# CVMI-Lab/HybridNeuralRendering

Hardware: AMD Instinct MI355X
Metric: rays/sec (fwd render) scene0241_01 at 1/2/4/8 GPU; PSNR delta vs ref (higher is better)
Workload: dtype f32

## Files before the change

hybridneuralrendering_amd/csrc/mlp.hip:

```cpp
#include <stdlib.h>

#include "hnr_h2.h"
#include "hnr_launch.h"

namespace hnr {

constexpr int ML_PAD = 32;
constexpr int ML_SLOT = 8192 + ML_PAD;
constexpr int ML_WSTEP = 8192;
constexpr int ML_META_FLOATS = 4 * 128 + 4 + 4;
constexpr int ML_DESC = 4 * 128, ML_WMAX = 4 * 128 + 4;

struct MlpArgs {
    const float *A; int lda;
    const float *R; const int32_t *ridx; int ldr;
    const char *wimg;
    int wbase[4];
    int K0, N[4], act[4];
    float *C2; int ldc2;
    const float *loc_w; const int32_t *vs_item;
    const float *w2c, *Kmat, *campos, *campos_n;
    const float *fm; int H, W;
    const float *frame_w;
    const float *w_last, *b_last;
// ... 712 lines not shown
    for (int i = tid; i < MX_WBYTES / 16; i += 64 * MX_WAVES) {
        const int s = i >> 8, cp = (i >> 6) & 3, ln = i & 63;
        *reinterpret_cast<u32x4 *>(lds + i * 16) = *reinterpret_cast<const u32x4 *>(a.wimg + (size_t)s * ML_WSTEP + cp * 1024 + ln * 16);
    }
    for (int i = tid; i < 3 * 64; i += 64 * MX_WAVES) s_bias[i] = meta[(i >> 6) * 128 + (i & 63)];
    for (int i = tid; i < 3 * 128; i += 64 * MX_WAVES) s_fin[i] = a.w_fin[i];
    __syncthreads();
    const float dw0 = meta[ML_DESC + 0], dw1 = meta[ML_DESC + 1], dw2 = meta[ML_DESC + 2];
    const float bfin[3] = {a.b_fin[0], a.b_fin[1], a.b_fin[2]};
    const f32x2 slope2 = {a.slope, a.slope};
    for (int tile = blockIdx.x * MX_WAVES + wave; tile < n_tiles; tile += gridDim.x * MX_WAVES) {
        int lane = tid & 63;
        asm volatile("" : "+v"(lane));
        const int h = lane >> 5, j = lane & 31;
        const long long sbase = (long long)tile * 32;
        if (h == 0) s_max[j] = 0u;
        MW_WAVE_FENCE();
        float inv;
        float4 f4[12];
#pragma unroll
        for (int it = 0; it < 12; ++it) {
            const int idx = lane + 64 * it, row = idx / 24, q = idx - row * 24;
            long long sidx = sbase + row;
            if (sidx >= n_samp) sidx = n_samp - 1;
            if (q < 23) {
                f4[it] = *reinterpret_cast<const float4 *>(a.X7 + (size_t)sidx * a.ld7 + 4 * q);
            } else f4[it] = make_float4(0.f, 0.f, 0.f, 0.f);
        }
#pragma unroll
        for (int it = 0; it < 12; ++it) {
            const int idx = lane + 64 * it, row = idx / 24, q = idx - row * 24;
            if (q == 22) { f4[it].z = 0.f; f4[it].w = 0.f; }
            const float m = fmaxf(fmaxf(fabsf(f4[it].x), fabsf(f4[it].y)), fmaxf(fabsf(f4[it].z), fabsf(f4[it].w)));
            atomicMax(s_max + row, __float_as_uint(m));
        }
        MW_WAVE_FENCE();
        auto planes_half = [&](int half) {
#pragma unroll
            for (int it = 0; it < 12; ++it) {
                const int idx = lane + 64 * it, row = idx / 24, q = idx - row * 24, c = 4 * q - 48 * half;
                if (c >= 0 && c < 48) {
                    const float sc = pow2f(row_scale_exp(__uint_as_float(s_max[row])));
                    unsigned ph0, pm0, ph1, pm1;
                    split2h(__fmul_rn(f4[it].x, sc), __fmul_rn(f4[it].y, sc), ph0, pm0);
                    split2h(__fmul_rn(f4[it].z, sc), __fmul_rn(f4[it].w, sc), ph1, pm1);
                    char *dst = wl + (c >> 4) * MW_SLOT + ((((c >> 3) & 1) * 32 + row) * 16) + (c & 7) * 2;
                    *reinterpret_cast<uint2 *>(dst) = make_uint2(ph0, ph1);
                    *reinterpret_cast<uint2 *>(dst + 1024) = make_uint2(pm0, pm1);
                }
            }
        };
        planes_half(0);
        inv = __fmul_rn(pow2f(-row_scale_exp(__uint_as_float(s_max[j]))), dw0);
        MW_WAVE_FENCE();
        f32x16 acc[2];
        auto zero_acc = [&]() {
#pragma unroll
            for (int c = 0; c < 2; ++c)
#pragma unroll
                for (int r = 0; r < 16; ++r) acc[c][r] = 0.f;
        };
        auto activate = [&](int layer, bool act) -> float {
            float m = 0.f;
            const f32x2 inv2 = {inv, inv};
#pragma unroll
            for (int c = 0; c < 2; ++c) {
#pragma unroll
                for (int q4 = 0; q4 < 4; ++q4) {
                    const float4 b = *reinterpret_cast<const float4 *>(s_bias + layer * 64 + 32 * c + 16 * h + 4 * q4);
#pragma unroll
                    for (int e = 0; e < 2; ++e) {
                        const int q = 2 * q4 + e;
                        const f32x2 add = e ? f32x2{b.z, b.w} : f32x2{b.x, b.y};
                        f32x2 v = f32x2_fma(f32x2{acc[c][2 * q], acc[c][2 * q + 1]}, inv2, add);
                        if (act) { const f32x2 sv = v * slope2; v.x = fmaxf(v.x, sv.x); v.y = fmaxf(v.y, sv.y); }
                        acc[c][2 * q] = v.x; acc[c][2 * q + 1] = v.y;
                        m = fmaxf(fmaxf(m, fabsf(v.x)), fabsf(v.y));
                    }
                }
            }
            return m;
        };
        auto publish = [&](float dw, float m) {
            m = fmaxf(m, __shfl_xor(m, 32));
            const int k = row_scale_exp(m);
            const float sc = pow2f(k);
            const f32x2 sc2 = {sc, sc};
            inv = __fmul_rn(pow2f(-k), dw);
            MW_WAVE_FENCE();
#pragma unroll
            for (int c = 0; c < 2; ++c) {
                unsigned ph[8], pm[8];
#pragma unroll
                for (int q = 0; q < 8; ++q) {
                    const f32x2 vs = f32x2{acc[c][2 * q], acc[c][2 * q + 1]} * sc2;
                    split2h(vs.x, vs.y, ph[q], pm[q]);
                }
                if (2 * c + h < 3) {
                    char *dst = wl + (2 * c + h) * MW_SLOT + j * 16;
                    *reinterpret_cast<u32x4 *>(dst) = u32x4{ph[0], ph[1], ph[2], ph[3]};
                    *reinterpret_cast<u32x4 *>(dst + 512) = u32x4{ph[4], ph[5], ph[6], ph[7]};
                    *reinterpret_cast<u32x4 *>(dst + 1024) = u32x4{pm[0], pm[1], pm[2], pm[3]};
                    *reinterpret_cast<u32x4 *>(dst + 1024 + 512) = u32x4{pm[4], pm[5], pm[6], pm[7]};
                }
            }
            MW_WAVE_FENCE();
        };
        const char *wp = lds + lane * 16, *bp = wl + lane * 16;
        long long srow = sbase + j;
        const bool ok = srow < n_samp;
        if (!ok) srow = n_samp - 1;
        zero_acc();
        mw_layer<3>(wp, bp, acc);
        MW_WAVE_FENCE();
        planes_half(1);
        MW_WAVE_FENCE();
        mw_layer<3>(wp + 3 * 4096, bp, acc);
        publish(dw1, activate(0, true));
        zero_acc();
        mw_layer<3>(wp + 6 * 4096, bp, acc);
        publish(dw2, activate(1, true));
        const float *cfrow = a.CF + (size_t)srow * a.ldcf;
        float4 cfa[2][4], cfb[8];
#pragma unroll
        for (int c = 0; c < 2; ++c)
#pragma unroll
            for (int q4 = 0; q4 < 4; ++q4) cfa[c][q4] = *reinterpret_cast<const float4 *>(cfrow + 32 * c + 16 * h + 4 * q4);
#pragma unroll
        for (int q4 = 0; q4 < 8; ++q4) cfb[q4] = *reinterpret_cast<const float4 *>(cfrow + 64 + 32 * h + 4 * q4);
        zero_acc();
        mw_layer<3>(wp + 9 * 4096, bp, acc);
        (void)activate(2, false);
        if (a.Y && ok) {
            float *o = a.Y + (size_t)srow * a.ldy;
#pragma unroll
            for (int c = 0; c < 2; ++c)
#pragma unroll
                for (int q4 = 0; q4 < 4; ++q4) {
                    const int col = 32 * c + 16 * h + 4 * q4;
                    if (col + 4 <= 48) *reinterpret_cast<float4 *>(o + col) = make_float4(acc[c][4 * q4], acc[c][4 * q4 + 1], acc[c][4 * q4 + 2], acc[c][4 * q4 + 3]);
                }
        }
        float x[2][16];
#pragma unroll
        for (int c = 0; c < 2; ++c)
#pragma unroll
            for (int r = 0; r < 16; ++r) {
                const float cfv = reinterpret_cast<const float *>(&cfa[c][0])[r];
                x[c][r] = (32 * c + 16 * h + r < 45) ? acc[c][r] + cfv : cfv;
            }
        float rj[3];
#pragma unroll
        for (int o = 0; o < 3; ++o) {
            const float *wf = s_fin + o * 128;
            float pa[2][2];
#pragma unroll
            for (int c = 0; c < 2; ++c)
#pragma unroll
                for (int hf = 0; hf < 2; ++hf) {
                    float r = 0.f;
#pragma unroll
                    for (int e = 0; e < 8; ++e) r += x[c][8 * hf + e] * wf[32 * c + 16 * h + 8 * hf + e];
                    pa[c][hf] = r;
                }
            float pb[4];
#pragma unroll
            for (int i = 0; i < 4; ++i) {
                float r = 0.f;
#pragma unroll
                for (int e = 0; e < 8; ++e) r += reinterpret_cast<const float *>(&cfb[0])[8 * i + e] * wf[64 + 32 * h + 8 * i + e];
                pb[i] = r;
            }
            const float u0 = pa[0][0] + pa[0][1];
            const float u1 = pa[1][0] + pa[1][1];
            const float uh = (pb[0] + pb[1]) + (pb[2] + pb[3]);
            const float v0 = __shfl_xor(u0, 32), v1 = __shfl_xor(u1, 32), vh = __shfl_xor(uh, 32);
            const float lo = (u0 + v0) + (v1 + u1);
            const float hi = vh + uh;
            rj[o] = lo + hi;
        }
        if (ok && h == 0) {
            float4 out;
            out.x = a.sigma[srow];
#pragma unroll
            for (int o = 0; o < 3; ++o) {
                const float sg = hnr_div(1.f, 1.f + expf(-(rj[o] + bfin[o])));
                const float cch = sg * (1.f + 2.f * 0.001f) - 0.001f;
                if (o == 0) out.y = cch; else if (o == 1) out.z = cch; else out.w = cch;
            }
            reinterpret_cast<float4 *>(a.decoded)[a.vs_item[srow]] = out;
        }
        MW_WAVE_FENCE();
    }
}

struct MlpPackArgs {
    const float *W[4]; int ldw[4], N[4], K[4], S[4], base[4];
    const float *b[4];
    char *out; int total_steps;
};

__global__ void mlp_wmax_kernel(MlpPackArgs a)
{
    const int l = blockIdx.y;
    unsigned *wmax = reinterpret_cast<unsigned *>(a.out + (size_t)a.total_steps * ML_WSTEP) + ML_WMAX;
    float m = 0.f;
    for (int i = blockIdx.x * blockDim.x + threadIdx.x; i < a.N[l] * a.K[l]; i += gridDim.x * blockDim.x) {
        const int n = i / a.K[l], k = i - n * a.K[l];
        m = fmaxf(m, fabsf(a.W[l][(size_t)n * a.ldw[l] + k]));
    }
    for (int o = 32; o > 0; o >>= 1) m = fmaxf(m, __shfl_xor(m, o));
    if ((threadIdx.x & 63) == 0) atomicMax(wmax + l, __float_as_uint(m));
}

__global__ void mlp_pack_kernel(MlpPackArgs a)
{
    const int l = blockIdx.y;
    float *meta = reinterpret_cast<float *>(a.out + (size_t)a.total_steps * ML_WSTEP);
    const unsigned maxbits = reinterpret_cast<const unsigned *>(meta)[ML_WMAX + l];
    int ex = (int)((maxbits >> 23) & 0xffu);
    ex = ex < 110 ? 110 : (ex > 160 ? 160 : ex);
    const int sw = CH_W_EXP + 126 - ex;
    const float scale = pow2f(sw);
    const int total = a.S[l] * 4 * 64 * 8;
    for (int i = blockIdx.x * blockDim.x + threadIdx.x; i < total; i += gridDim.x * blockDim.x) {
        const int e = i & 7, ln = (i >> 3) & 63, ct = (i >> 9) & 3, s = i >> 11;
        const int ii = ln & 31, hh = ln >> 5;
        const int n = 32 * ct + 16 * ((ii >> 2) & 1) + (ii & 3) + 4 * (ii >> 3), k = 16 * s + 8 * hh + e;
        const float x = (n < a.N[l] && k < a.K[l]) ? __fmul_rn(a.W[l][(size_t)n * a.ldw[l] + k], scale) : 0.f;
        const _Float16 hv = (_Float16)x;
        const _Float16 mv = (_Float16)__fsub_rn(x, (float)hv);
        _Float16 *dst = reinterpret_cast<_Float16 *>(a.out + a.base[l] + (size_t)s * ML_WSTEP + (ct * 2) * 1024 + ln * 16) + e;
        dst[0] = hv;
        dst[512] = mv;
    }
    if (blockIdx.x == 0) {
        for (int i = threadIdx.x; i < 128; i += blockDim.x) meta[l * 128 + i] = (a.b[l] && i < a.N[l]) ? a.b[l][i] : 0.f;
        if (threadIdx.x == 0) meta[ML_DESC + l] = pow2f(-sw);
    }
}

}

using namespace hnr;

static int mlp_steps(int K) { return (K + 15) / 16; }

extern "C" int64_t hnr_mlp3_packed_bytes(int n_layers, const int *K)
{
    if (!K || (n_layers != 3 && n_layers != 4)) return -1;
    int64_t steps = 0;
    for (int l = 0; l < n_layers; ++l) { if (K[l] <= 0 || K[l] > 288) return -1; steps += mlp_steps(K[l]); }
    return steps * ML_WSTEP + ML_META_FLOATS * 4;
}

extern "C" int hnr_mlp3_pack(int n_layers, const float *const *d_W, const int *ldw, const int *N, const int *K, const float *const *d_bias, void *d_packed,
                             void *stream)
{
    if ((n_layers != 3 && n_layers != 4) || !d_W || !ldw || !N || !K || !d_bias || !d_packed || ((uintptr_t)d_packed & 15)) { set_error("hnr_mlp3_pack: NULL / unaligned pointer or n_layers not 3 / 4"); return HNR_ERR_BADARG; }
    MlpPackArgs a;
    int steps = 0;
    for (int l = 0; l < n_layers; ++l) {
        if (!d_W[l] || N[l] <= 0 || N[l] > 128 || K[l] <= 0 || K[l] > 288 || ldw[l] < K[l] || (l > 0 && K[l] != N[l == 3 ? 2 : l - 1])) {
            set_error("hnr_mlp3_pack: layer %d: N=%d (1..128) K=%d (1..288, = N of the layer it reads) ldw=%d", l, N[l], K[l], ldw[l]);
            return HNR_ERR_BADARG;
        }
        a.W[l] = d_W[l]; a.ldw[l] = ldw[l]; a.N[l] = N[l]; a.K[l] = K[l]; a.S[l] = mlp_steps(K[l]); a.b[l] = d_bias[l];
        a.base[l] = steps * ML_WSTEP;
        steps += a.S[l];
    }
    a.out = (char *)d_packed; a.total_steps = steps;
    hipStream_t st = (hipStream_t)stream;
    HNR_HIP_CHECK(hipMemsetAsync(a.out + (size_t)steps * ML_WSTEP, 0, ML_META_FLOATS * 4, st));
    mlp_wmax_kernel<<<dim3(16, n_layers), 256, 0, st>>>(a);
    HNR_LAUNCH_CHECK();
    mlp_pack_kernel<<<dim3(32, n_layers), 256, 0, st>>>(a);
    HNR_LAUNCH_CHECK();
    return HNR_OK;
}

static void mlp3_probe_print(hipStream_t st, int n_layers, int K0)
{
#ifdef HNR_MLP_PROBE
    if (knob_now("HNR_MLP_PROBE_PRINT", 0)) {
        (void)hipStreamSynchronize(st);
        long long h[24];
        if (hipMemcpyFromSymbol(h, HIP_SYMBOL(g_mlp_probe), sizeof(h)) == hipSuccess && h[20] > 0) {
            const char *nm[13] = {"wait/prev", "A load + split", "barrier", "L0 mfma", "L0 act", "L0 publish", "L1 mfma+act", "L1 publish", "L2 mfma", "L2 act", "store", "tail", "end barrier"};
            fprintf(stderr, "[mlp3 probe] n_layers %d K0 %d tiles %lld:", n_layers, K0, h[20]);
            for (int i = 0; i < 13; ++i) fprintf(stderr, " %s %lld", nm[i], h[i] / h[20]);
            fprintf(stderr, " [merge (a) %lld | tail: dot %lld, sigmoid %lld, loads %lld, merge+stores %lld]", h[13] / h[20], h[14] / h[20], h[15] / h[20], h[16] / h[20], h[17] / h[20]);
            fprintf(stderr, "\n");
        }
    }
#else
    (void)st; (void)n_layers; (void)K0;
#endif
}

static int mlp3_forward_impl(const float *d_A, int lda, int64_t M_cap, const int64_t *d_counts, int count_index, int count_mult, int seg_stride,
                             const void *d_packed, int n_layers, const int *N, const int *K, const int *act, float slope, const float *d_R,
                             const int32_t *d_ridx, int ldr, float *d_C, int ldc, float *d_C2, int ldc2, float *d_T0, int ldt0, float *d_T1, int ldt1,
                             uint32_t *d_tmax, void *stream);

extern "C" int hnr_mlp3_forward(const float *d_A, int lda, int64_t M_cap, const int64_t *d_counts, int count_index, int count_mult, int seg_stride,
                                const void *d_packed, int n_layers, const int *N, const int *K, const int *act, float slope, const float *d_R,
                                const int32_t *d_ridx, int ldr, float *d_C, int ldc, float *d_C2, int ldc2, void *stream)
{
    return mlp3_forward_impl(d_A, lda, M_cap, d_counts, count_index, count_mult, seg_stride, d_packed, n_layers, N, K, act, slope, d_R, d_ridx, ldr, d_C, ldc,
                             d_C2, ldc2, nullptr, 0, nullptr, 0, nullptr, stream);
}

namespace hnr {
int mlp3_forward_train(const float *d_A, int lda, int64_t M_cap, const int64_t *d_counts, int count_index, int count_mult, int seg_stride,
                       const void *d_packed, int n_layers, const int *N, const int *K, const int *act, float slope, const float *d_R,
                       const int32_t *d_ridx, int ldr, float *d_C, int ldc, float *d_C2, int ldc2, float *d_T0, int ldt0, float *d_T1, int ldt1,
                       uint32_t *d_tmax, void *stream)
{
    if (!d_T0 || !d_T1 || ldt0 < N[0] || ldt1 < N[1] || (ldt0 & 3) || (ldt1 & 3) || ((uintptr_t)d_T0 & 15) || ((uintptr_t)d_T1 & 15)) { set_error("mlp3_forward_train: bad activation buffers"); return HNR_ERR_BADARG; }
    return mlp3_forward_impl(d_A, lda, M_cap, d_counts, count_index, count_mult, seg_stride, d_packed, n_layers, N, K, act, slope, d_R, d_ridx, ldr, d_C, ldc,
                             d_C2, ldc2, d_T0, ldt0, d_T1, ldt1, d_tmax, stream);
}
}

static int mlp3_forward_impl(const float *d_A, int lda, int64_t M_cap, const int64_t *d_counts, int count_index, int count_mult, int seg_stride,
                             const void *d_packed, int n_layers, const int *N, const int *K, const int *act, float slope, const float *d_R,
                             const int32_t *d_ridx, int ldr, float *d_C, int ldc, float *d_C2, int ldc2, float *d_T0, int ldt0, float *d_T1, int ldt1,
                             uint32_t *d_tmax, void *stream)
{
    if ((n_layers != 3 && n_layers != 4) || !N || !K || !act || M_cap < 0 || seg_stride < 0 || (seg_stride > 0 && (count_mult < 1 || count_mult > 8)) || lda < K[0] || (lda & 3) || ldc < N[2] || (ldc & 3) ||
        !(slope > 0.f && slope < 1.f) || (d_R && (!d_ridx || ldr < N[0] || (ldr & 3) || ((uintptr_t)d_R & 15))) || (n_layers == 4 && (!d_C2 || ldc2 < N[3] || (ldc2 & 3) || ((uintptr_t)d_C2 & 15)))) {
        set_error("hnr_mlp3_forward: bad sizes (n_layers=%d lda=%d ldc=%d ldr=%d ldc2=%d slope=%g)", n_layers, lda, ldc, ldr, ldc2, (double)slope);
        return HNR_ERR_BADARG;
    }
    if (M_cap == 0) return HNR_OK;
    if (!d_A || !d_packed || !d_C || ((uintptr_t)d_A & 15) || ((uintptr_t)d_C & 15) || ((uintptr_t)d_packed & 15) || ((uintptr_t)d_R & 7)) {
        set_error("hnr_mlp3_forward: NULL / unaligned pointer");
        return HNR_ERR_BADARG;
    }
    MlpArgs a;
    a.A = d_A; a.lda = lda; a.R = d_R; a.ridx = d_ridx; a.ldr = ldr; a.wimg = (const char *)d_packed;
    int steps = 0, S[4] = {0, 0, 0, 0};
    a.N[3] = 0; a.act[3] = 0; a.wbase[3] = 0;
    for (int l = 0; l < n_layers; ++l) {
        if (N[l] <= 0 || N[l] > 128 || K[l] <= 0 || K[l] > 288 || (l > 0 && K[l] != N[l == 3 ? 2 : l - 1])) { set_error("hnr_mlp3_forward: bad layer %d (N=%d K=%d)", l, N[l], K[l]); return HNR_ERR_BADARG; }
        S[l] = mlp_steps(K[l]); a.wbase[l] = steps * ML_WSTEP; steps += S[l]; a.N[l] = N[l]; a.act[l] = act[l];
    }
    a.K0 = K[0]; a.slope = slope;
    a.counts = reinterpret_cast<const unsigned long long *>(d_counts); a.count_index = count_index; a.count_mult = count_mult; a.M_cap = M_cap;
    a.seg_stride = seg_stride;
    a.C = d_C; a.ldc = ldc; a.C2 = d_C2; a.ldc2 = ldc2;
    a.T0 = d_T0; a.ldt0 = ldt0; a.T1 = d_T1; a.ldt1 = ldt1; a.tmax = d_tmax;
    a.loc_w = nullptr; a.vs_item = nullptr; a.w2c = a.Kmat = a.campos = a.campos_n = a.fm = a.frame_w = a.w_last = a.b_last = a.CF = nullptr;
    a.H = a.W = a.ldcf = a.ld7 = 0; a.X7 = nullptr;
    const int n_cu = device_num_cus();
    hipStream_t st = (hipStream_t)stream;
#define HNR_MLP3_CASE(S0_, S1_, S2_, S3_, RT_)                                                                                         \
    if (S[0] == S0_ && S[1] == S1_ && S[2] == S2_ && S[3] == S3_) {                                                                     \
        if (S1_ <= 4 && S2_ <= 4 && S3_ == 0 && RT_ >= 2 && N[2] > 64) {    \
            set_error("hnr_mlp3_forward: N[2] = %d > 64 with 64-wide hidden layers is not built", N[2]); return HNR_ERR_BADARG; }             \
        constexpr int smax3 = S0_ > S1_ ? (S0_ > S2_ ? S0_ : S2_) : (S1_ > S2_ ? S1_ : S2_), smax = smax3 > S3_ ? smax3 : S3_;          \
        constexpr int ldsb = smax * (RT_ * 2048 + ML_PAD) + 32 * RT_ * 4 * 4 + 32 * RT_ * 4;                                                       \
        const int64_t tiles = (M_cap + 32 * RT_ - 1) / (32 * RT_);                                                                      \
        const int wgs = mlp3_wgs_per_cu(S0_, RT_, 0) * n_cu, grid = (int)(tiles < wgs ? tiles : wgs);                                              \
        const int rc = launch_lds<mlp3_kernel<S0_, S1_, S2_, S3_, 0, RT_>>(grid, 256, ldsb, st, a);                                        \
        mlp3_probe_print(st, n_layers, K[0]);                                                                                          \
        return rc;                                                                                                                      \
    }
    HNR_MLP3_CASE(18, 8, 8, 0, 2)
    HNR_MLP3_CASE(18, 8, 8, 8, 2)
    HNR_MLP3_CASE(3, 4, 4, 0, 4)
    HNR_MLP3_CASE(6, 3, 3, 0, 2)
#undef HNR_MLP3_CASE
    set_error("hnr_mlp3_forward: no kernel for k steps (%d, %d, %d, %d); built: (18,8,8,0) (18,8,8,8) (3,4,4,0) (6,3,3,0)", S[0], S[1], S[2], S[3]);
    return HNR_ERR_BADARG;
}


extern "C" int hnr_merge_stage(const float *d_sample_loc_w, const int32_t *d_vs_item, const int64_t *d_counts, const float *d_w2c, const float *d_intrinsic,
                               const float *d_campos, const float *d_campos_nearest, const float *d_featmap, int V, int H, int W, const float *d_frame_w,
                               const float *d_pre, int ldpre, const void *d_mlp_mw, const float *d_w_last, const float *d_b_last, const float *d_CF, int ldcf,
                               int cap_samples, float slope, float *d_X7, int ld7, void *stream)
{
    if (V != 4) { set_error("hnr_merge_stage: built for V = 4 reference views (got %d); use hnr_proj_rows + hnr_mlp3_forward + hnr_merge", V); return HNR_ERR_BADARG; }
    if (cap_samples < 0 || H <= 0 || W <= 0 || ldpre < 64 || (ldpre & 3) || ((uintptr_t)d_pre & 15) || ldcf < 45 || ld7 < 90 || !(slope > 0.f && slope < 1.f)) {
        set_error("hnr_merge_stage: bad sizes (cap_samples=%d H=%d W=%d ldpre=%d ldcf=%d ld7=%d)", cap_samples, H, W, ldpre, ldcf, ld7); return HNR_ERR_BADARG;
    }
    if (cap_samples == 0) return HNR_OK;
    if (!d_sample_loc_w || !d_vs_item || !d_counts || !d_w2c || !d_intrinsic || !d_campos || !d_campos_nearest || !d_featmap || !d_pre || !d_mlp_mw ||
        !d_w_last || !d_b_last || !d_CF || !d_X7 || ((uintptr_t)d_featmap & 15) || ((uintptr_t)d_pre & 7) || ((uintptr_t)d_mlp_mw & 15)) {
        set_error("hnr_merge_stage: NULL / unaligned pointer"); return HNR_ERR_BADARG;
    }
    MlpArgs a;
    a.A = nullptr; a.lda = 48; a.R = d_pre; a.ridx = nullptr; a.ldr = ldpre; a.wimg = (const char *)d_mlp_mw;
    a.wbase[0] = 0; a.wbase[1] = 3 * ML_WSTEP; a.wbase[2] = 7 * ML_WSTEP; a.wbase[3] = 0;
    a.K0 = 48; a.N[0] = a.N[1] = a.N[2] = 64; a.N[3] = 0; a.act[0] = a.act[1] = a.act[2] = 1; a.act[3] = 0;
    a.slope = slope;
    a.counts = reinterpret_cast<const unsigned long long *>(d_counts); a.count_index = HNR_CNT_SAMPLES_VALID; a.count_mult = 4; a.M_cap = (long long)cap_samples * 4;
    a.seg_stride = 0; a.C = nullptr; a.ldc = 64; a.C2 = nullptr; a.ldc2 = 0;
    a.T0 = a.T1 = nullptr; a.ldt0 = a.ldt1 = 0; a.tmax = nullptr;
    a.loc_w = d_sample_loc_w; a.vs_item = d_vs_item; a.w2c = d_w2c; a.Kmat = d_intrinsic; a.campos = d_campos; a.campos_n = d_campos_nearest;
    a.fm = d_featmap; a.H = H; a.W = W; a.frame_w = d_frame_w; a.w_last = d_w_last; a.b_last = d_b_last; a.CF = d_CF; a.ldcf = ldcf; a.X7 = d_X7; a.ld7 = ld7;
    const int n_cu = device_num_cus();
    static const int rt_env = knob("HNR_MERGE_RT", 1);
    const int rt_sel = rt_env == 4 || rt_env == 2 ? rt_env : 1;
    const bool wp_ok = ldcf >= 48 && !(ldcf & 3) && !((uintptr_t)d_CF & 15) && ld7 >= 92 && !(ld7 & 3) && !((uintptr_t)d_X7 & 15);
    if (rt_sel == 1 && wp_ok) {
        const int64_t wtiles = ((int64_t)cap_samples + 7) / 8, wg_tiles = (wtiles + MW_WAVES - 1) / MW_WAVES;
        const int g = (int)(wg_tiles < (int64_t)n_cu ? wg_tiles : (int64_t)n_cu);
        return launch_lds<merge_wp_kernel>(g, 64 * MW_WAVES, MW_LDS, (hipStream_t)stream, a);
    }
    const int rt_k = rt_sel == 4 ? 4 : 2;
    const int rows = 32 * rt_k, wgs = mlp3_wgs_per_cu(3, rt_k, 1);
    const int64_t tiles = ((int64_t)cap_samples * 4 + rows - 1) / rows;
    const int grid = (int)(tiles < (int64_t)wgs * n_cu ? tiles : (int64_t)wgs * n_cu);
    const int ldsb = 4 * (rt_k * 2048 + ML_PAD) + rows * 4 * 4 + rows * 4 + rows * 48 * 4 + 3 * rows * 4 + 128 * 4;
    const int rc = rt_k == 4 ? launch_lds<mlp3_kernel<3, 4, 4, 0, 1, 4>>(grid, 256, ldsb, (hipStream_t)stream, a)
                             : launch_lds<mlp3_kernel<3, 4, 4, 0, 1, 2>>(grid, 256, ldsb, (hipStream_t)stream, a);
    mlp3_probe_print((hipStream_t)stream, 3, 48);
    return rc;
}

extern "C" int hnr_mixup_stage(const float *d_X7, int ld7, const void *d_mlp_mx, const float *d_CF, int ldcf, const float *d_w_fin, const float *d_b_fin,
                               const float *d_sigma, const int32_t *d_vs_item, const int64_t *d_counts, int cap_samples, float slope, float *d_Y, int ldy,
                               float *d_decoded, void *stream)
{
    if (cap_samples < 0 || ld7 < 92 || (ld7 & 3) || ldcf < 128 || (ldcf & 3) || (d_Y && (ldy < 48 || (ldy & 3))) || !(slope > 0.f && slope < 1.f)) {
        set_error("hnr_mixup_stage: bad sizes (cap_samples=%d ld7=%d ldcf=%d ldy=%d)", cap_samples, ld7, ldcf, ldy); return HNR_ERR_BADARG;
    }
    if (cap_samples == 0) return HNR_OK;
    if (!d_X7 || !d_mlp_mx || !d_CF || !d_w_fin || !d_b_fin || !d_sigma || !d_vs_item || !d_counts || !d_decoded || ((uintptr_t)d_X7 & 15) ||
        ((uintptr_t)d_CF & 15) || ((uintptr_t)d_mlp_mx & 15) || ((uintptr_t)d_Y & 15) || ((uintptr_t)d_decoded & 15)) {
        set_error("hnr_mixup_stage: NULL / unaligned pointer"); return HNR_ERR_BADARG;
    }
    MixArgs a;
    a.X7 = d_X7; a.ld7 = ld7; a.wimg = (const char *)d_mlp_mx; a.CF = d_CF; a.ldcf = ldcf; a.w_fin = d_w_fin; a.b_fin = d_b_fin; a.sigma = d_sigma;
    a.vs_item = d_vs_item; a.counts = reinterpret_cast<const unsigned long long *>(d_counts); a.S_cap = cap_samples; a.slope = slope;
    a.Y = d_Y; a.ldy = ldy; a.decoded = d_decoded;
    const int n_cu = device_num_cus();
    const int64_t tiles = ((int64_t)cap_samples + 31) / 32, wg_tiles = (tiles + MX_WAVES - 1) / MX_WAVES;
    const int g = (int)(wg_tiles < (int64_t)n_cu ? wg_tiles : (int64_t)n_cu);
    return launch_lds<mixfinal_wp_kernel>(g, 64 * MX_WAVES, MX_LDS, (hipStream_t)stream, a);
}
```

Measured before the change: 8.250 million.

## Add specialized fused MLP kernel for 280-input 128-wide color/feature network

Adds a dedicated kernel for the common 280→128→128→128 (+optional 64-wide linear tail) MLP shape, dispatched by default when the layer shape, strides and flags match. It hardcodes the layout with compile-time constants, loads 64-row tiles via buffer loads with out-of-range rows masked, and chains the three or four layers through LDS with per-row power-of-two rescaling and split-half MFMA. The aim is to cut generic-kernel overhead such as runtime shape handling, probes and residual paths for the hot shape. It adds a second code path to maintain, and correctness depends on the shape guard matching exactly.

```diff
diff --git a/hybridneuralrendering_amd/csrc/cf.hip b/hybridneuralrendering_amd/csrc/cf.hip
--- /dev/null
+++ b/hybridneuralrendering_amd/csrc/cf.hip
@@ -0,0 +1,213 @@
+#include "hnr_h2.h"
+#include "hnr_launch.h"
+
+namespace hnr {
+
+constexpr int CF_WSTEP = 8192, CF_DESC = 4 * 128;
+constexpr int CF_S0 = 18, CF_S1 = 8;
+constexpr int CF_ROWS = 64;
+constexpr int CF_SLOT = 2 * 2048 + 32;
+constexpr int CF_LDA = 280 * 4, CF_LDC = 128 * 4, CF_LDP = 64 * 4;
+constexpr int CF_O_EXCH = CF_S0 * CF_SLOT;
+constexpr int CF_O_RINV = CF_O_EXCH + CF_ROWS * 16;
+constexpr int CF_O_BIAS = CF_O_RINV + CF_ROWS * 4;
+constexpr int CF_LDS = CF_O_BIAS + 4 * 128 * 4;
+constexpr unsigned CF_DROP = 0x40000000u;
+
+typedef float f32x4m __attribute__((ext_vector_type(4)));
+
+struct CfArgs {
+    const float *A;
+    const char *wimg;
+    float *C, *C2;
+    const unsigned long long *counts; int count_index, count_mult; long long M_cap;
+    float slope;
+};
+
+#define CF_LDS_BARRIER() asm volatile("s_waitcnt lgkmcnt(0)\n\ts_barrier" ::: "memory")
+#define CF_RSRC(p_, n_) __builtin_amdgcn_make_buffer_rsrc(const_cast<char *>(reinterpret_cast<const char *>(p_)), 0, (n_), 0x00020000)
+
+template <int TAIL>
+__global__ __launch_bounds__(256, 2) void cf_kernel(CfArgs a)
+{
+    constexpr int STEPS = CF_S0 + 2 * CF_S1 + TAIL * CF_S1;
+    constexpr int WB1 = CF_S0 * CF_WSTEP, WB2 = WB1 + CF_S1 * CF_WSTEP, WB3 = WB2 + CF_S1 * CF_WSTEP, META = STEPS * CF_WSTEP;
+    extern __shared__ __attribute__((aligned(16))) char lds[];
+    const int wave0 = __builtin_amdgcn_readfirstlane((int)threadIdx.x >> 6);
+    long long M = a.M_cap;
+    if (a.counts) { const long long c = (long long)a.counts[a.count_index] * a.count_mult; if (c < M) M = c; }
+    const int n_tiles = (int)((M + CF_ROWS - 1) / CF_ROWS);
+    const __amdgpu_buffer_rsrc_t wsrd = CF_RSRC(a.wimg, META);
+    const float *meta = reinterpret_cast<const float *>(a.wimg + META);
+    for (int i = threadIdx.x; i < 4 * 128; i += 256) *reinterpret_cast<float *>(lds + CF_O_BIAS + 4 * i) = (TAIL || i < 3 * 128) ? meta[i] : 0.f;
+    const float dw0 = meta[CF_DESC + 0], dw1 = meta[CF_DESC + 1], dw2 = meta[CF_DESC + 2], dw3 = TAIL ? meta[CF_DESC + 3] : 0.f;
+    const float slope = a.slope;
+    __syncthreads();
+
+    for (int tile = blockIdx.x; tile < n_tiles; tile += gridDim.x) {
+        int tid = threadIdx.x, wave = wave0;
+        asm volatile("" : "+v"(tid));
+        asm volatile("" : "+s"(wave));
+        const int lane = tid & 63, h = lane >> 5, j = lane & 31;
+        const long long row_base = (long long)tile * CF_ROWS;
+        const long long left = M - row_base;
+        const int nv = left < CF_ROWS ? (int)left : CF_ROWS;
+        const __amdgpu_buffer_rsrc_t xrs = CF_RSRC(reinterpret_cast<const char *>(a.A) + row_base * CF_LDA, nv * CF_LDA);
+        const __amdgpu_buffer_rsrc_t crs = CF_RSRC(reinterpret_cast<char *>(a.C) + row_base * CF_LDC, nv * CF_LDC);
+        const __amdgpu_buffer_rsrc_t prs = CF_RSRC(reinterpret_cast<char *>(a.C2) + row_base * CF_LDP, TAIL ? nv * CF_LDP : 0);
+
+        {
+            const int lr = lane & 15, sub = lane >> 4;
+            const int lr4 = lr < 8 ? lr : 6 + (lr & 1);
+            const unsigned drop4 = lr < 6 ? 0u : CF_DROP;
+            f32x4m v[4][5];
+#pragma unroll
+            for (int b = 0; b < 4; ++b) {
+                const int rl = 16 * wave + 4 * b + sub;
+                const int rc = rl < nv ? rl : nv - 1;
+                const unsigned voff = __umul24((unsigned)rc, (unsigned)CF_LDA) + (unsigned)lr * 16u;
+#pragma unroll
+                for (int nb = 0; nb < 4; ++nb) v[b][nb] = __builtin_bit_cast(f32x4m, __builtin_amdgcn_raw_buffer_load_b128(xrs, voff + nb * 256, 0, 0));
+                v[b][4] = __builtin_bit_cast(f32x4m, __builtin_amdgcn_raw_buffer_load_b128(xrs, (voff | drop4) + 1024, 0, 0));
+            }
+#pragma unroll
+            for (int b = 0; b < 4; ++b) {
+                const int rl = 16 * wave + 4 * b + sub;
+                float m = 0.f;
+#pragma unroll
+                for (int nb = 0; nb < 5; ++nb)
+#pragma unroll
+                    for (int e = 0; e < 4; ++e) m = fmaxf(m, fabsf(v[b][nb][e]));
+                m = fmaxf(m, __builtin_amdgcn_update_dpp(m, m, 0xB1, 0xf, 0xf, false));
+                m = fmaxf(m, __builtin_amdgcn_update_dpp(m, m, 0x4E, 0xf, 0xf, false));
+                m = fmaxf(m, __builtin_amdgcn_update_dpp(m, m, 0x141, 0xf, 0xf, false));
+                m = fmaxf(m, __builtin_amdgcn_update_dpp(m, m, 0x140, 0xf, 0xf, false));
+                const int k = row_scale_exp(m);
+                const float sc = pow2f(k);
+                *reinterpret_cast<float *>(lds + CF_O_RINV + 4 * rl) = pow2f(-k);
+#pragma unroll
+                for (int nb = 0; nb < 5; ++nb) {
+                    const int c = 4 * (nb * 16 + (nb < 4 ? lr : lr4));
+                    unsigned ph0, pm0, ph1, pm1;
+                    split2h(__fmul_rn(v[b][nb][0], sc), __fmul_rn(v[b][nb][1], sc), ph0, pm0);
+                    split2h(__fmul_rn(v[b][nb][2], sc), __fmul_rn(v[b][nb][3], sc), ph1, pm1);
+                    char *dst = lds + (c >> 4) * CF_SLOT + ((rl >> 5) * 2) * 1024 + ((((c >> 3) & 1) * 32 + (rl & 31)) * 16) + (c & 7) * 2;
+                    *reinterpret_cast<uint2 *>(dst) = make_uint2(ph0, ph1);
+                    *reinterpret_cast<uint2 *>(dst + 1024) = make_uint2(pm0, pm1);
+                }
+            }
+        }
+        CF_LDS_BARRIER();
+
+        const int col0 = 32 * wave + 16 * h;
+        const unsigned woff = (unsigned)wave * 2048u + (unsigned)lane * 16u;
+        float inv[2];
+#pragma unroll
+        for (int rt = 0; rt < 2; ++rt) inv[rt] = __fmul_rn(*reinterpret_cast<const float *>(lds + CF_O_RINV + 4 * (32 * rt + j)), dw0);
+        f32x16 acc[2][1];
+        auto zero_acc = [&]() {
+#pragma unroll
+            for (int rt = 0; rt < 2; ++rt)
+#pragma unroll
+                for (int r = 0; r < 16; ++r) acc[rt][0][r] = 0.f;
+        };
+        float amax[2];
+        auto activate = [&](int layer) {
+            f32x4m bias[4];
+#pragma unroll
+            for (int q = 0; q < 4; ++q) bias[q] = *reinterpret_cast<const f32x4m *>(lds + CF_O_BIAS + (layer * 128 + col0 + 4 * q) * 4);
+#pragma unroll
+            for (int rt = 0; rt < 2; ++rt) {
+                float m = 0.f;
+#pragma unroll
+                for (int r = 0; r < 16; ++r) {
+                    float x = fmaf(acc[rt][0][r], inv[rt], bias[r >> 2][r & 3]);
+                    x = fmaxf(x, __fmul_rn(x, slope));
+                    acc[rt][0][r] = x;
+                    m = fmaxf(m, fabsf(x));
+                }
+                amax[rt] = m;
+            }
+        };
+        auto publish = [&](float dw) {
+#pragma unroll
+            for (int rt = 0; rt < 2; ++rt) {
+                const float m = fmaxf(amax[rt], __shfl_xor(amax[rt], 32));
+                *reinterpret_cast<float *>(lds + CF_O_EXCH + ((32 * rt + j) * 4 + wave) * 4) = m;
+            }
+            CF_LDS_BARRIER();
+#pragma unroll
+            for (int rt = 0; rt < 2; ++rt) {
+                const f32x4m m4 = *reinterpret_cast<const f32x4m *>(lds + CF_O_EXCH + (32 * rt + j) * 16);
+                const int k = row_scale_exp(fmaxf(fmaxf(m4[0], m4[1]), fmaxf(m4[2], m4[3])));
+                const float sc = pow2f(k);
+                inv[rt] = __fmul_rn(pow2f(-k), dw);
+                unsigned ph[8], pm[8];
+#pragma unroll
+                for (int q = 0; q < 8; ++q) split2h(__fmul_rn(acc[rt][0][2 * q], sc), __fmul_rn(acc[rt][0][2 * q + 1], sc), ph[q], pm[q]);
+                char *dst = lds + (2 * wave + h) * CF_SLOT + (rt * 2) * 1024 + j * 16;
+                *reinterpret_cast<u32x4 *>(dst) = u32x4{ph[0], ph[1], ph[2], ph[3]};
+                *reinterpret_cast<u32x4 *>(dst + 512) = u32x4{ph[4], ph[5], ph[6], ph[7]};
+                *reinterpret_cast<u32x4 *>(dst + 1024) = u32x4{pm[0], pm[1], pm[2], pm[3]};
+                *reinterpret_cast<u32x4 *>(dst + 1024 + 512) = u32x4{pm[4], pm[5], pm[6], pm[7]};
+            }
+            CF_LDS_BARRIER();
+        };
+
+        zero_acc();
+        h2_mfma_layer<2, 1, CF_S0, 0, CF_WSTEP, CF_SLOT>(wsrd, 0, woff, lds, lane, acc, []() {});
+        activate(0);
+        publish(dw1);
+        zero_acc();
+        h2_mfma_layer<2, 1, CF_S1, 0, CF_WSTEP, CF_SLOT>(wsrd, WB1, woff, lds, lane, acc, []() {});
+        activate(1);
+        publish(dw2);
+        zero_acc();
+        h2_mfma_layer<2, 1, CF_S1, 0, CF_WSTEP, CF_SLOT>(wsrd, WB2, woff, lds, lane, acc, []() {});
+        activate(2);
+        {
+            const unsigned co = (unsigned)j * CF_LDC + (unsigned)col0 * 4u;
+#pragma unroll
+            for (int rt = 0; rt < 2; ++rt)
+#pragma unroll
+                for (int q = 0; q < 4; ++q)
+                    __builtin_amdgcn_raw_buffer_store_b128(u32x4{__float_as_uint(acc[rt][0][4 * q]), __float_as_uint(acc[rt][0][4 * q + 1]), __float_as_uint(acc[rt][0][4 * q + 2]),
+                                                                 __float_as_uint(acc[rt][0][4 * q + 3])}, crs, co + rt * 32 * CF_LDC + q * 16, 0, 0);
+        }
+        if (TAIL) {
+            publish(dw3);
+            const int ct = wave & 1, rtt = wave >> 1;
+            const int colt = 32 * ct + 16 * h;
+            const float invt = rtt ? inv[1] : inv[0];
+            f32x16 acct[1][1];
+#pragma unroll
+            for (int r = 0; r < 16; ++r) acct[0][0][r] = 0.f;
+            h2_mfma_layer<1, 1, CF_S1, 0, CF_WSTEP, CF_SLOT>(wsrd, WB3, (unsigned)ct * 2048u + (unsigned)lane * 16u, lds + rtt * 2048, lane, acct, []() {});
+            const unsigned po = (unsigned)(32 * rtt + j) * CF_LDP + (unsigned)colt * 4u;
+#pragma unroll
+            for (int q = 0; q < 4; ++q) {
+                const f32x4m b = *reinterpret_cast<const f32x4m *>(lds + CF_O_BIAS + (3 * 128 + colt + 4 * q) * 4);
+                u32x4 o;
+#pragma unroll
+                for (int e = 0; e < 4; ++e) o[e] = __float_as_uint(fmaf(acct[0][0][4 * q + e], invt, b[e]));
+                __builtin_amdgcn_raw_buffer_store_b128(o, prs, po + q * 16, 0, 0);
+            }
+        }
+        CF_LDS_BARRIER();
+    }
+}
+
+int cf_forward(const float *d_A, int64_t M_cap, const int64_t *d_counts, int count_index, int count_mult, const void *d_packed, float slope, float *d_C,
+               float *d_C2, void *stream)
+{
+    if (M_cap == 0) return HNR_OK;
+    CfArgs a;
+    a.A = d_A; a.wimg = (const char *)d_packed; a.C = d_C; a.C2 = d_C2;
+    a.counts = reinterpret_cast<const unsigned long long *>(d_counts); a.count_index = count_index; a.count_mult = count_mult; a.M_cap = M_cap;
+    a.slope = slope;
+    const int64_t tiles = (M_cap + CF_ROWS - 1) / CF_ROWS;
+    const int wgs = 2 * device_num_cus(), grid = (int)(tiles < wgs ? tiles : wgs);
+    return d_C2 ? launch_lds<cf_kernel<1>>(grid, 256, CF_LDS, (hipStream_t)stream, a) : launch_lds<cf_kernel<0>>(grid, 256, CF_LDS, (hipStream_t)stream, a);
+}
+
+}
diff --git a/hybridneuralrendering_amd/csrc/mlp.hip b/hybridneuralrendering_amd/csrc/mlp.hip
--- a/hybridneuralrendering_amd/csrc/mlp.hip
+++ b/hybridneuralrendering_amd/csrc/mlp.hip
@@ -1038,6 +1038,10 @@
                              const void *d_packed, int n_layers, const int *N, const int *K, const int *act, float slope, const float *d_R,
                              const int32_t *d_ridx, int ldr, float *d_C, int ldc, float *d_C2, int ldc2, float *d_T0, int ldt0, float *d_T1, int ldt1,
                              uint32_t *d_tmax, void *stream);
+namespace hnr {
+int cf_forward(const float *d_A, int64_t M_cap, const int64_t *d_counts, int count_index, int count_mult, const void *d_packed, float slope, float *d_C,
+               float *d_C2, void *stream);
+}
 
 extern "C" int hnr_mlp3_forward(const float *d_A, int lda, int64_t M_cap, const int64_t *d_counts, int count_index, int count_mult, int seg_stride,
                                 const void *d_packed, int n_layers, const int *N, const int *K, const int *act, float slope, const float *d_R,
@@ -1089,6 +1093,9 @@
     a.T0 = d_T0; a.ldt0 = ldt0; a.T1 = d_T1; a.ldt1 = ldt1; a.tmax = d_tmax;
     a.loc_w = nullptr; a.vs_item = nullptr; a.w2c = a.Kmat = a.campos = a.campos_n = a.fm = a.frame_w = a.w_last = a.b_last = a.CF = nullptr;
     a.H = a.W = a.ldcf = a.ld7 = 0; a.X7 = nullptr;
+    if (S[0] == 18 && K[0] == 280 && lda == 280 && N[0] == 128 && N[1] == 128 && N[2] == 128 && ldc == 128 && act[0] && act[1] && act[2] &&
+        (n_layers == 3 || (N[3] == 64 && ldc2 == 64 && !act[3])) && !d_R && seg_stride == 0 && !d_T0 && !d_T1 && !d_tmax && knob_now("HNR_CF_KERNEL", 1))
+        return cf_forward(d_A, M_cap, d_counts, count_index, count_mult, d_packed, slope, d_C, n_layers == 4 ? d_C2 : nullptr, stream);
     const int n_cu = device_num_cus();
     hipStream_t st = (hipStream_t)stream;
 #define HNR_MLP3_CASE(S0_, S1_, S2_, S3_, RT_)                                                                                         \
```

Result: no change. 8.286 million, median of 6 (+0.4%).
